# JokerYan/MS-GS

Measured on AMD Instinct MI355X. Metric: Mpixels/s fwd+bwd @1080p, 1M Gaussians; fraction of HBM roofline, higher is better.
Workload: dtype f32

## Files before the change

### ms-gs_amd/csrc/preprocess.hip

```cpp
#include "msgs_internal.h"

#include <type_traits>

#pragma clang fp contract(off)

namespace msgs {

namespace {

constexpr float SH_C0 = 0.28209479177387814f;
constexpr float SH_C1 = 0.4886025119029199f;
__device__ constexpr float SH_C2[5] = {1.0925484305920792f, -1.0925484305920792f, 0.31539156525252005f,
                                       -1.0925484305920792f, 0.5462742152960396f};
__device__ constexpr float SH_C3[7] = {-0.5900435899266435f, 2.890611442640554f, -0.4570457994644658f,
                                       0.3731763325901154f, -0.4570457994644658f, 1.445305721320277f,
                                       -0.5900435899266435f};

struct Cam {
    float V[16];
    float M[16];
    float cam[3];
};

__device__ __forceinline__ void load_cam(const ViewParams& vp, Cam& c) {
#pragma unroll
    for (int i = 0; i < 16; ++i) { c.V[i] = vp.viewmatrix[i]; c.M[i] = vp.projmatrix[i]; }
#pragma unroll
    for (int i = 0; i < 3; ++i) c.cam[i] = vp.campos[i];
}

__device__ __forceinline__ void cov3d_from_scale_rot(const float* s, float mod, const float* q, float* cov) {
    const float r = q[0], x = q[1], y = q[2], z = q[3];
    const float R[3][3] = {{1.f - 2.f * (y * y + z * z), 2.f * (x * y - r * z), 2.f * (x * z + r * y)},
                           {2.f * (x * y + r * z), 1.f - 2.f * (x * x + z * z), 2.f * (y * z - r * x)},
                           {2.f * (x * z - r * y), 2.f * (y * z + r * x), 1.f - 2.f * (x * x + y * y)}};
    const float S[3] = {mod * s[0], mod * s[1], mod * s[2]};
    float M[3][3];
#pragma unroll
    for (int i = 0; i < 3; ++i)
#pragma unroll
        for (int j = 0; j < 3; ++j) M[i][j] = R[i][j] * S[j];
    cov[0] = M[0][0] * M[0][0] + M[0][1] * M[0][1] + M[0][2] * M[0][2];
    cov[1] = M[0][0] * M[1][0] + M[0][1] * M[1][1] + M[0][2] * M[1][2];
    cov[2] = M[0][0] * M[2][0] + M[0][1] * M[2][1] + M[0][2] * M[2][2];
    cov[3] = M[1][0] * M[1][0] + M[1][1] * M[1][1] + M[1][2] * M[1][2];
    cov[4] = M[1][0] * M[2][0] + M[1][1] * M[2][1] + M[1][2] * M[2][2];
    cov[5] = M[2][0] * M[2][0] + M[2][1] * M[2][1] + M[2][2] * M[2][2];
}

struct Cov2D {
    float T[2][3];
    float a, b, c;
    float tx_c, ty_c, tz, x_mul, y_mul;
};

__device__ __forceinline__ void compute_cov2d(const float* t, const ViewParams& vp, const float* cov3D,
                                              const float* V, Cov2D& o) {
    const float limx = 1.3f * vp.tanfovx, limy = 1.3f * vp.tanfovy;
    const float txtz = t[0] / t[2], tytz = t[1] / t[2];
    o.x_mul = (txtz < -limx || txtz > limx) ? 0.f : 1.f;
    o.y_mul = (tytz < -limy || tytz > limy) ? 0.f : 1.f;
    o.tx_c = fminf(limx, fmaxf(-limx, txtz)) * t[2];
    o.ty_c = fminf(limy, fmaxf(-limy, tytz)) * t[2];
    o.tz = t[2];
    const float J[2][3] = {{vp.fx / t[2], 0.f, -(vp.fx * o.tx_c) / (t[2] * t[2])},
                           {0.f, vp.fy / t[2], -(vp.fy * o.ty_c) / (t[2] * t[2])}};
#pragma unroll
    for (int r = 0; r < 2; ++r)
#pragma unroll
        for (int c = 0; c < 3; ++c)
            o.T[r][c] = J[r][0] * V[4 * c + 0] + J[r][1] * V[4 * c + 1] + J[r][2] * V[4 * c + 2];
    const float S[3][3] = {{cov3D[0], cov3D[1], cov3D[2]}, {cov3D[1], cov3D[3], cov3D[4]},
                           {cov3D[2], cov3D[4], cov3D[5]}};
    float ST[2][3];
#pragma unroll
    for (int r = 0; r < 2; ++r)
#pragma unroll
        for (int i = 0; i < 3; ++i) ST[r][i] = S[i][0] * o.T[r][0] + S[i][1] * o.T[r][1] + S[i][2] * o.T[r][2];
    o.a = (o.T[0][0] * ST[0][0] + o.T[0][1] * ST[0][1] + o.T[0][2] * ST[0][2]) + 0.3f;
    o.b = o.T[0][0] * ST[1][0] + o.T[0][1] * ST[1][1] + o.T[0][2] * ST[1][2];
    o.c = (o.T[1][0] * ST[1][0] + o.T[1][1] * ST[1][1] + o.T[1][2] * ST[1][2]) + 0.3f;
}

__device__ __forceinline__ void view_point(const float* V, const float* p, float* t) {
    t[0] = ((V[0] * p[0] + V[4] * p[1]) + V[8] * p[2]) + V[12];
    t[1] = ((V[1] * p[0] + V[5] * p[1]) + V[9] * p[2]) + V[13];
    t[2] = ((V[2] * p[0] + V[6] * p[1]) + V[10] * p[2]) + V[14];
}

__device__ __forceinline__ void proj_point(const float* M, const float* p, float* h) {
#pragma unroll
    for (int k = 0; k < 4; ++k) h[k] = ((M[k] * p[0] + M[4 + k] * p[1]) + M[8 + k] * p[2]) + M[12 + k];
}

__device__ __forceinline__ float pixel_size_of(float opacity, float conA, float conC) {
    const float v = 255.0f * opacity;
    if (!(v > 1.0f) || !(conA > 0.f) || !(conC > 0.f)) return 0.f;
    const float ell = 2.0f * logf(v);
    const float sx = 2.0f * sqrtf(ell / conA);
    const float sy = 2.0f * sqrtf(ell / conC);
    return fminf(sx, sy);
}

__device__ __forceinline__ float filter_weight(const ViewParams& vp, float size, float minps, float maxps,
                                               bool base) {
    float w = 1.0f;
    if (vp.filter_small && !base && minps > 0.f && size < minps) {
        if (vp.fade_size > 0.f) {
            const float rel = minps / fmaxf(size, 1e-30f);
            w *= fminf(1.f, fmaxf(0.f, 1.f - (rel - 1.f) / vp.fade_size));
        } else w = 0.f;
    }
    if (vp.filter_large && maxps > 0.f && size > maxps) {
        if (vp.fade_size > 0.f) {
            const float rel = size / maxps;
            w *= fminf(1.f, fmaxf(0.f, 1.f - (rel - 1.f) / vp.fade_size));
        } else w = 0.f;
    }
    return w;
}

__device__ __forceinline__ float sh_channel(int deg, const float* sh, int c, float x, float y, float z) {
    auto S = [&](int k) { return sh[k * 3 + c]; };
    float r = SH_C0 * S(0);
    if (deg > 0) {
        r = r - SH_C1 * y * S(1) + SH_C1 * z * S(2) - SH_C1 * x * S(3);
        if (deg > 1) {
            const float xx = x * x, yy = y * y, zz = z * z, xy = x * y, yz = y * z, xz = x * z;
            r = r + SH_C2[0] * xy * S(4) + SH_C2[1] * yz * S(5) + SH_C2[2] * (2.0f * zz - xx - yy) * S(6) +
                SH_C2[3] * xz * S(7) + SH_C2[4] * (xx - yy) * S(8);
            if (deg > 2) {
                r = r + SH_C3[0] * y * (3.0f * xx - yy) * S(9) + SH_C3[1] * xy * z * S(10) +
                    SH_C3[2] * y * (4.0f * zz - xx - yy) * S(11) +
                    SH_C3[3] * z * (2.0f * zz - 3.0f * xx - 3.0f * yy) * S(12) +
                    SH_C3[4] * x * (4.0f * zz - xx - yy) * S(13) + SH_C3[5] * z * (xx - yy) * S(14) +
                    SH_C3[6] * x * (xx - 3.0f * yy) * S(15);
            }
        }
    }
    return r;
}


__device__ __forceinline__ void sh_basis(int deg, float x, float y, float z, float b[16]) {
#pragma unroll
    for (int k = 0; k < 16; ++k) b[k] = 0.f;
    b[0] = SH_C0;
    if (deg > 0) {
        b[1] = -(SH_C1 * y); b[2] = SH_C1 * z; b[3] = -(SH_C1 * x);
        if (deg > 1) {
            const float xx = x * x, yy = y * y, zz = z * z, xy = x * y, yz = y * z, xz = x * z;
            b[4] = SH_C2[0] * xy; b[5] = SH_C2[1] * yz; b[6] = SH_C2[2] * (2.0f * zz - xx - yy);
            b[7] = SH_C2[3] * xz; b[8] = SH_C2[4] * (xx - yy);
            if (deg > 2) {
                b[9] = SH_C3[0] * y * (3.0f * xx - yy); b[10] = SH_C3[1] * xy * z;
                b[11] = SH_C3[2] * y * (4.0f * zz - xx - yy);
                b[12] = SH_C3[3] * z * (2.0f * zz - 3.0f * xx - 3.0f * yy);
                b[13] = SH_C3[4] * x * (4.0f * zz - xx - yy); b[14] = SH_C3[5] * z * (xx - yy);
                b[15] = SH_C3[6] * x * (xx - 3.0f * yy);
            }
        }
    }
}

template <int K_LO, int K_HI, class F>
__device__ __forceinline__ void sh_coef_table(int deg, float x, float y, float z, F&& coef) {
    auto at = [&](int k, float basis, float bx, float by, float bz) {
        if (k >= K_LO && k < K_HI) coef(k, basis, bx, by, bz);
    };
    at(0, SH_C0, 0.f, 0.f, 0.f);
    if (deg > 0) {
        at(1, -SH_C1 * y, 0.f, -SH_C1, 0.f);
        at(2, SH_C1 * z, 0.f, 0.f, SH_C1);
        at(3, -SH_C1 * x, -SH_C1, 0.f, 0.f);
        if (deg > 1) {
            const float xx = x * x, yy = y * y, zz = z * z, xy = x * y, yz = y * z, xz = x * z;
            at(4, SH_C2[0] * xy, SH_C2[0] * y, SH_C2[0] * x, 0.f);
            at(5, SH_C2[1] * yz, 0.f, SH_C2[1] * z, SH_C2[1] * y);
            at(6, SH_C2[2] * (2.f * zz - xx - yy), SH_C2[2] * -2.f * x, SH_C2[2] * -2.f * y, SH_C2[2] * 4.f * z);
            at(7, SH_C2[3] * xz, SH_C2[3] * z, 0.f, SH_C2[3] * x);
            at(8, SH_C2[4] * (xx - yy), SH_C2[4] * 2.f * x, SH_C2[4] * -2.f * y, 0.f);
            if (deg > 2) {
                at(9, SH_C3[0] * y * (3.f * xx - yy), SH_C3[0] * 6.f * xy, SH_C3[0] * (3.f * xx - 3.f * yy), 0.f);
                at(10, SH_C3[1] * xy * z, SH_C3[1] * yz, SH_C3[1] * xz, SH_C3[1] * xy);
                at(11, SH_C3[2] * y * (4.f * zz - xx - yy), SH_C3[2] * -2.f * xy, SH_C3[2] * (4.f * zz - xx - 3.f * yy), SH_C3[2] * 8.f * yz);
                at(12, SH_C3[3] * z * (2.f * zz - 3.f * xx - 3.f * yy), SH_C3[3] * -6.f * xz, SH_C3[3] * -6.f * yz, SH_C3[3] * (6.f * zz - 3.f * xx - 3.f * yy));
                at(13, SH_C3[4] * x * (4.f * zz - xx - yy), SH_C3[4] * (4.f * zz - 3.f * xx - yy), SH_C3[4] * -2.f * xy, SH_C3[4] * 8.f * xz);
                at(14, SH_C3[5] * z * (xx - yy), SH_C3[5] * 2.f * xz, SH_C3[5] * -2.f * yz, SH_C3[5] * (xx - yy));
                at(15, SH_C3[6] * x * (xx - 3.f * yy), SH_C3[6] * (3.f * xx - 3.f * yy), SH_C3[6] * -6.f * xy, 0.f);
            }
        }
    }
}

__device__ __forceinline__ bool sh_jacobian_stored(const msgs_gaussians_t& g, const ViewParams& vp) {
    return g.raw_params != 0 || (g.shs != nullptr && vp.sh_coeffs == 16);
}

struct ShJacobian { float j[3][3]; };


template <int K_LO, int K_HI, int K_ROW>
__device__ __forceinline__ void sh_colour_accumulate(float* rgb, ShJacobian& J, int deg, float x, float y, float z,
                                                     const float* row) {
    sh_coef_table<K_LO, K_HI>(deg, x, y, z, [&](int k, float basis, float bx, float by, float bz) {
#pragma unroll
        for (int c = 0; c < 3; ++c) {
            const float v = row[3 * (k - K_ROW) + c];
            rgb[c] = rgb[c] + basis * v;
            J.j[c][0] = fmaf(bx, v, J.j[c][0]);
            J.j[c][1] = fmaf(by, v, J.j[c][1]);
            J.j[c][2] = fmaf(bz, v, J.j[c][2]);
        }
    });
}

__device__ __forceinline__ void sh_jacobian_store(char* geom, const GeomLayout& L, int P, int i, const ShJacobian& J) {
    float4* pl = reinterpret_cast<float4*>(geom + L.shjac);
    pl[i] = make_float4(J.j[0][0], J.j[0][1], J.j[0][2], J.j[1][0]);
    pl[(size_t)P + i] = make_float4(J.j[1][1], J.j[1][2], J.j[2][0], J.j[2][1]);
    reinterpret_cast<float*>(pl + 2 * (size_t)P)[i] = J.j[2][2];
}

__device__ __forceinline__ void sh_jacobian_load(const char* geom, const GeomLayout& L, int P, int i, ShJacobian& J) {
    const float4* pl = reinterpret_cast<const float4*>(geom + L.shjac);
    const float4 a = pl[i], b = pl[(size_t)P + i];
    J.j[0][0] = a.x; J.j[0][1] = a.y; J.j[0][2] = a.z; J.j[1][0] = a.w;
    J.j[1][1] = b.x; J.j[1][2] = b.y; J.j[2][0] = b.z; J.j[2][1] = b.w;
    J.j[2][2] = reinterpret_cast<const float*>(pl + 2 * (size_t)P)[i];
}

__device__ __forceinline__ void sh_ddir_from_jacobian(const ShJacobian& J, const float* g, float* ddir) {
#pragma unroll
    for (int j = 0; j < 3; ++j) ddir[j] = fmaf(J.j[2][j], g[2], fmaf(J.j[1][j], g[1], J.j[0][j] * g[0]));
}

struct ViewDir { float x, y, z, len; };
__device__ __forceinline__ ViewDir view_dir(const float* p, const float* campos) {
    const float dox = p[0] - campos[0], doy = p[1] - campos[1], doz = p[2] - campos[2];
    const float len = sqrtf(dox * dox + doy * doy + doz * doz);
    return {dox / len, doy / len, doz / len, len};
}

__device__ __forceinline__ void direction_backward(const ViewDir& d, const float* ddir, float* dm) {
    const float dotv = d.x * ddir[0] + d.y * ddir[1] + d.z * ddir[2];
    dm[0] = (ddir[0] - d.x * dotv) / d.len;
    dm[1] = (ddir[1] - d.y * dotv) / d.len;
    dm[2] = (ddir[2] - d.z * dotv) / d.len;
}

__device__ __forceinline__ void clamp_mask(float* dcolr, uint32_t fl) {
#pragma unroll
    for (int c = 0; c < 3; ++c)
        if (fl & (1u << c)) dcolr[c] = 0.f;
}

__device__ __forceinline__ void wave_lds_fence() {
    __builtin_amdgcn_fence(__ATOMIC_RELEASE, "wavefront");
    __builtin_amdgcn_wave_barrier();
    __builtin_amdgcn_fence(__ATOMIC_ACQUIRE, "wavefront");
}

constexpr int ROW_F = 48;
constexpr int ROW_LDS = 49;
constexpr int K9_STAGE_ROWS = 32;

__device__ __forceinline__ int sh_row_float4s(int deg) { return deg == 0 ? 1 : deg == 1 ? 3 : deg == 2 ? 7 : 12; }

constexpr int HALF_F4 = 6;
constexpr int HALF_LDS = 25;
__device__ __forceinline__ void coop_load_rows_part(float* lds_rows, const float* g_rows, const uint8_t* idx, int nrow,
                                                    int f4_first, int n4, int lane) {
    const int rpi = 64 / n4;
    const int sub = lane / n4, c = lane - sub * n4;
    for (int it = 0; it * rpi < nrow; ++it) {
        const int slot = it * rpi + sub;
        if (sub < rpi && slot < nrow) {
            const int sl = idx[slot];
            const float4 v = *reinterpret_cast<const float4*>(g_rows + (size_t)sl * ROW_F + 4 * (f4_first + c));
            float* d = lds_rows + sl * HALF_LDS + 4 * c;
            d[0] = v.x; d[1] = v.y; d[2] = v.z; d[3] = v.w;
        }
    }
}

__device__ __forceinline__ void coop_store_rows(const float* lds_rows, float* g_rows, int nrow, uint64_t live,
                                                int nfloat, int lane, bool acc) {
    constexpr int n4 = ROW_F / 4, rpi = 64 / n4;
    const int sub = lane / n4, c = lane - sub * n4;
    for (int it = 0; it * rpi < nrow; ++it) {
        const int row = it * rpi + sub;
        if (sub < rpi && row < nrow) {
            const bool on = (live >> row) & 1ull;
            if (acc && !on) continue;
            float4 v = make_float4(0.f, 0.f, 0.f, 0.f);
            if (on) {
                const float* sp = lds_rows + row * ROW_LDS + 4 * c;
                v.x = 4 * c + 0 < nfloat ? sp[0] : 0.f;
                v.y = 4 * c + 1 < nfloat ? sp[1] : 0.f;
                v.z = 4 * c + 2 < nfloat ? sp[2] : 0.f;
                v.w = 4 * c + 3 < nfloat ? sp[3] : 0.f;
            }
            float4* dst = reinterpret_cast<float4*>(g_rows + (size_t)row * ROW_F + 4 * c);
            if (acc) { const float4 o = *dst; v.x = o.x + v.x; v.y = o.y + v.y; v.z = o.z + v.z; v.w = o.w + v.w; }
            *dst = v;
        }
    }
}

constexpr int REST_F = 45;

__device__ __forceinline__ float act_opacity(const msgs_gaussians_t& g, int i) {
    const float x = g.opacities[i];
    return g.raw_params == 1 ? 1.0f / (1.0f + expf(-x)) : x;
}
__device__ __forceinline__ void act_scales(const msgs_gaussians_t& g, int i, float* s) {
#pragma unroll
    for (int k = 0; k < 3; ++k) { const float x = g.scales[3 * i + k]; s[k] = g.raw_params == 1 ? expf(x) : x; }
}
__device__ __forceinline__ float act_rotation(const msgs_gaussians_t& g, int i, float* q) {
    const float4 q4 = reinterpret_cast<const float4*>(g.rotations)[i];
    q[0] = q4.x; q[1] = q4.y; q[2] = q4.z; q[3] = q4.w;
    if (g.raw_params == 0) return 1.0f;
    if (g.raw_params == 2) {
        const float4 r4 = reinterpret_cast<const float4*>(g.rotations_raw)[i];
        return sqrtf(r4.x * r4.x + r4.y * r4.y + r4.z * r4.z + r4.w * r4.w);
    }
    const float rn = sqrtf(q[0] * q[0] + q[1] * q[1] + q[2] * q[2] + q[3] * q[3]);
    const float n = fmaxf(rn, 1e-12f);
#pragma unroll
    for (int k = 0; k < 4; ++k) q[k] = q[k] / n;
    return rn;
}
__device__ __forceinline__ void normalize_backward(const float* q, float rn, float* dq) {
    const float n = fmaxf(rn, 1e-12f);
    const float dotq = rn < 1e-12f ? 0.f : q[0] * dq[0] + q[1] * dq[1] + q[2] * dq[2] + q[3] * dq[3];
#pragma unroll
    for (int k = 0; k < 4; ++k) dq[k] = (dq[k] - q[k] * dotq) / n;
}

typedef float msgs_f3 __attribute__((ext_vector_type(3)));
typedef msgs_f3 __attribute__((aligned(4))) msgs_f3_u;
__device__ __forceinline__ void coop_load_split_half_listed(float* lds_rows, const float* dc, const float* rest, int wave_first,
                                                            const uint8_t* idx, int nlisted, int half, int lane) {
    const int sub = lane >> 3, c = lane & 7;
    for (int it = 0; it * 8 < nlisted; ++it) {
        const int slot = it * 8 + sub;
        if (slot < nlisted) {
            const int sl = idx[slot];
            const size_t gi = (size_t)wave_first + sl;
            float* d = lds_rows + sl * HALF_LDS + 3 * c;
            const float* src = (half == 0 && c == 0) ? dc + gi * 3 : rest + gi * 45 + 3 * (8 * half + c - 1);
            const msgs_f3 v = *reinterpret_cast<const msgs_f3_u*>(src);
            d[0] = v.x; d[1] = v.y; d[2] = v.z;
        }
    }
}

__device__ __forceinline__ void coop_load_split_rows(float* lds_rows, const float* dc, const float* rest, int i,
                                                     bool in_range, int wave_first, int nrow, int lane, int lrow) {
    if (in_range) {
#pragma unroll
        for (int c = 0; c < 3; ++c) lds_rows[lrow * ROW_LDS + c] = dc[3 * (size_t)i + c];
    }
    const float* src = rest + (size_t)wave_first * REST_F;
    const int nflat = nrow * REST_F;
    for (int base = 0; base < nflat; base += 256) {
        const int f0 = base + lane * 4;
        float v[4] = {0.f, 0.f, 0.f, 0.f};
        if (f0 + 3 < nflat) {
            const float4 t = *reinterpret_cast<const float4*>(src + f0);
            v[0] = t.x; v[1] = t.y; v[2] = t.z; v[3] = t.w;
        } else {
#pragma unroll
            for (int j = 0; j < 4; ++j) if (f0 + j < nflat) v[j] = src[f0 + j];
        }
#pragma unroll
        for (int j = 0; j < 4; ++j) {
            const int f = f0 + j;
            if (f < nflat) { const int row = f / REST_F; lds_rows[row * ROW_LDS + 3 + (f - row * REST_F)] = v[j]; }
        }
    }
}

__device__ __forceinline__ void coop_store_split_rows(const float* lds_rows, float* d_dc, float* d_rest, int i,
                                                      bool in_range, int wave_first, int nrow, uint64_t live,
                                                      int nfloat, int lane, int lrow, bool acc = false) {
    if (in_range) {
        const bool on = (live >> lrow) & 1ull;
        if (!acc) {
#pragma unroll
            for (int c = 0; c < 3; ++c) d_dc[3 * (size_t)i + c] = on ? lds_rows[lrow * ROW_LDS + c] : 0.f;
        } else if (on) {
#pragma unroll
            for (int c = 0; c < 3; ++c) d_dc[3 * (size_t)i + c] = d_dc[3 * (size_t)i + c] + lds_rows[lrow * ROW_LDS + c];
        }
    }
    float* dst = d_rest + (size_t)wave_first * REST_F;
    const int nflat = nrow * REST_F;
    for (int base = 0; base < nflat; base += 256) {
        const int f0 = base + lane * 4;
        float v[4];
        bool on[4];
#pragma unroll
        for (int j = 0; j < 4; ++j) {
            const int f = min(f0 + j, nflat - 1);
            const int row = f / REST_F, k = f - row * REST_F;
            on[j] = (live >> row) & 1ull;
            v[j] = (on[j] && 3 + k < nfloat) ? lds_rows[row * ROW_LDS + 3 + k] : 0.f;
        }
        if (f0 + 3 < nflat) {
            float4* d4 = reinterpret_cast<float4*>(dst + f0);
            if (!acc) {
                *d4 = make_float4(v[0], v[1], v[2], v[3]);
            } else if (on[0] || on[3]) {
                const float4 o = *d4;
                *d4 = make_float4(o.x + v[0], o.y + v[1], o.z + v[2], o.w + v[3]);
            }
        } else {
#pragma unroll
            for (int j = 0; j < 4; ++j)
                if (f0 + j < nflat) {
                    if (!acc) dst[f0 + j] = v[j];
                    else if (on[j]) dst[f0 + j] = dst[f0 + j] + v[j];
                }
        }
    }
}

__device__ __forceinline__ void coop_adam_split_rows(const float* lds_rows, float* p_dc, float* p_rest, const AdamInBackward& ad,
                                                     int i, bool in_range, int wave_first, int nrow, uint64_t live,
                                                     int nfloat, int lane, int lrow) {
    if (in_range) {
        const bool on = (live >> lrow) & 1ull;
#pragma unroll
        for (int c = 0; c < 3; ++c) {
            const size_t at = 3 * (size_t)i + c;
            float p = p_dc[at], m = ad.m[1][at], v = ad.v[1][at];
            adam_update(p, on ? lds_rows[lrow * ROW_LDS + c] : 0.f, m, v, ad.nss[1], ad.a);
            p_dc[at] = p; ad.m[1][at] = m; ad.v[1][at] = v;
        }
    }
    const size_t off = (size_t)wave_first * REST_F;
    float* __restrict__ P = p_rest + off;
    float* __restrict__ M = ad.m[2] + off;
    float* __restrict__ V = ad.v[2] + off;
    const float nss = ad.nss[2];
    const int nflat = nrow * REST_F;
    for (int base = 0; base < nflat; base += 256) {
        const int f0 = base + lane * 4;
        float g[4];
#pragma unroll
        for (int j = 0; j < 4; ++j) {
            const int f = min(f0 + j, nflat - 1);
            const int row = f / REST_F, k = f - row * REST_F;
            g[j] = (((live >> row) & 1ull) && 3 + k < nfloat) ? lds_rows[row * ROW_LDS + 3 + k] : 0.f;
        }
        if (f0 + 3 < nflat) {
            float4 p = *reinterpret_cast<const float4*>(P + f0), m = *reinterpret_cast<const float4*>(M + f0),
                   v = *reinterpret_cast<const float4*>(V + f0);
            adam_update(p.x, g[0], m.x, v.x, nss, ad.a);
            adam_update(p.y, g[1], m.y, v.y, nss, ad.a);
            adam_update(p.z, g[2], m.z, v.z, nss, ad.a);
            adam_update(p.w, g[3], m.w, v.w, nss, ad.a);
            *reinterpret_cast<float4*>(P + f0) = p;
            *reinterpret_cast<float4*>(M + f0) = m;
            *reinterpret_cast<float4*>(V + f0) = v;
        } else {
#pragma unroll
            for (int j = 0; j < 4; ++j)
                if (f0 + j < nflat) {
                    float p = P[f0 + j], m = M[f0 + j], v = V[f0 + j];
                    adam_update(p, g[j], m, v, nss, ad.a);
                    P[f0 + j] = p; M[f0 + j] = m; V[f0 + j] = v;
                }
        }
    }
}

template <bool SPLIT_ROWS>
__global__ __launch_bounds__(256) __attribute__((amdgpu_waves_per_eu(6))) void preprocess_kernel(ViewParams vp, msgs_gaussians_t g,
                                                         int32_t* __restrict__ radii,
                                                         float* __restrict__ pixel_sizes,
                                                         char* __restrict__ geom, ZeroJob zj,
                                                         uint32_t* __restrict__ heavy_list,
                                                         uint32_t* __restrict__ heavy_count,
                                                         uint32_t* __restrict__ heavy_blk, int write_litrec) {
    __shared__ float s_rows[4][64 * HALF_LDS];
    __shared__ uint8_t s_idx[4][64];
    __shared__ uint32_t s_heavy[4], s_hvw[4];
    const int P = g.P;
    {
        const size_t t0 = (size_t)blockIdx.x * blockDim.x + threadIdx.x, nt = (size_t)gridDim.x * blockDim.x;
        for (size_t t = t0; t < zj.n0; t += nt) zj.p0[t] = 0u;
        for (size_t t = t0; t < zj.n1; t += nt) zj.p1[t] = 0u;
    }
    const int i = blockIdx.x * blockDim.x + threadIdx.x;
    const int lane = threadIdx.x & 63, wv = threadIdx.x >> 6;
    const bool in_range = i < P;
    const GeomLayout L(P);
    GaussRec* rec = reinterpret_cast<GaussRec*>(geom + L.rec);
    BinRec* binrec = reinterpret_cast<BinRec*>(geom + L.binrec);
    uint32_t* tiles = reinterpret_cast<uint32_t*>(geom + L.tiles);
    uint32_t* key = reinterpret_cast<uint32_t*>(geom + L.key);
    uint32_t* flags = reinterpret_cast<uint32_t*>(geom + L.flags);
    float* weight = reinterpret_cast<float*>(geom + L.weight);

    Cam cm;
    load_cam(vp, cm);

    int32_t out_radius = 0;
    float out_psize = 0.f;
    uint32_t out_tiles = 0, out_cells = 0, out_key = 0xFFFFFFFFu, out_flags = 0;
    float out_weight = 0.f, out_tau2 = -3.0e38f;

    bool alive = false;
    float p[3] = {0.f, 0.f, 1.f}, t[3] = {0.f, 0.f, 0.f};
    float conA = 0.f, conB = 0.f, conC = 0.f, px = 0.f, py = 0.f, my_radius = 0.f, w = 0.f, o_eff = 0.f;
    int minx = 0, miny = 0, maxx = 0, maxy = 0;
    if (in_range) {
        p[0] = g.means3D[3 * i]; p[1] = g.means3D[3 * i + 1]; p[2] = g.means3D[3 * i + 2];
        view_point(cm.V, p, t);
    }
    do {
        if (!in_range || t[2] <= 0.2f) break;
        float h[4];
        proj_point(cm.M, p, h);
        const float pw = 1.0f / (h[3] + 0.0000001f);
        const float ndc_x = h[0] * pw, ndc_y = h[1] * pw;
        float cov3D[6];
        if (g.cov3D_precomp) {
#pragma unroll
            for (int k = 0; k < 6; ++k) cov3D[k] = g.cov3D_precomp[6 * i + k];
        } else {
            float sc[3], q[4];
            act_scales(g, i, sc);
            act_rotation(g, i, q);
            cov3d_from_scale_rot(sc, vp.scale_modifier, q, cov3D);
        }
        Cov2D c2;
        compute_cov2d(t, vp, cov3D, cm.V, c2);
        const float det = c2.a * c2.c - c2.b * c2.b;
        if (det == 0.0f) break;
        const float det_inv = 1.f / det;
        conA = c2.c * det_inv; conB = -c2.b * det_inv; conC = c2.a * det_inv;
        const float mid = 0.5f * (c2.a + c2.c);
        const float root = sqrtf(fmaxf(0.1f, mid * mid - det));
        const float lam1 = mid + root, lam2 = mid - root;
        my_radius = ceilf(3.f * sqrtf(fmaxf(lam1, lam2)));
        px = ((ndc_x + 1.0f) * vp.W - 1.0f) * 0.5f;
        py = ((ndc_y + 1.0f) * vp.H - 1.0f) * 0.5f;
        const float o = act_opacity(g, i);
        out_psize = pixel_size_of(o, conA, conC);
        minx = min(vp.gx, max(0, (int)((px - my_radius) / TILE)));
        miny = min(vp.gy, max(0, (int)((py - my_radius) / TILE)));
        maxx = min(vp.gx, max(0, (int)((px + my_radius + TILE - 1) / TILE)));
        maxy = min(vp.gy, max(0, (int)((py + my_radius + TILE - 1) / TILE)));
        if ((maxx - minx) * (maxy - miny) == 0) break;
        w = filter_weight(vp, out_psize, g.min_pixel_sizes ? g.min_pixel_sizes[i] : -1.f,
                          g.max_pixel_sizes ? g.max_pixel_sizes[i] : -1.f,
                          g.base_mask ? g.base_mask[i] != 0 : false);
        if (!(w > 0.f)) break;
        o_eff = o * w;
        alive = true;
    } while (false);

    const bool raw = g.raw_params != 0;
    const bool split_in = SPLIT_ROWS && raw && g.shs == nullptr;
    const bool staged_sh = sh_jacobian_stored(g, vp);
    float rgb[3] = {0.f, 0.f, 0.f};
    float dirx = 0.f, diry = 0.f, dirz = 0.f;
    if (alive) {
        const ViewDir d = view_dir(p, cm.cam);
        dirx = d.x; diry = d.y; dirz = d.z;
    }
    if (staged_sh) {
        const uint64_t need = __ballot(alive);
        if (alive) s_idx[wv][__popcll(need & ((1ull << lane) - 1ull))] = (uint8_t)lane;
        const int wave_first = blockIdx.x * blockDim.x + wv * 64;
        const int n4_total = sh_row_float4s(vp.sh_degree);
        ShJacobian J = {};
        for (int half = 0; half * HALF_F4 < n4_total; ++half) {
            wave_lds_fence();
            if (split_in) {
                if (need != 0)
                    coop_load_split_half_listed(s_rows[wv], g.features_dc, g.features_rest, wave_first, s_idx[wv], __popcll(need),
                                                half, lane);
            } else {
                coop_load_rows_part(s_rows[wv], g.shs + (size_t)wave_first * ROW_F, s_idx[wv], __popcll(need),
                                    half * HALF_F4, min(HALF_F4, n4_total - half * HALF_F4), lane);
            }
            wave_lds_fence();
            if (alive) {
                const float* row = (const float*)&s_rows[wv][lane * HALF_LDS];
                asm volatile("" : "+v"(dirx), "+v"(diry), "+v"(dirz));
                if (half == 0) {
                    sh_colour_accumulate<0, 4, 0>(rgb, J, vp.sh_degree, dirx, diry, dirz, row);
                    __builtin_amdgcn_sched_barrier(0);
                    sh_colour_accumulate<4, 8, 0>(rgb, J, vp.sh_degree, dirx, diry, dirz, row);
                } else {
                    sh_colour_accumulate<8, 12, 8>(rgb, J, vp.sh_degree, dirx, diry, dirz, row);
                    __builtin_amdgcn_sched_barrier(0);
                    sh_colour_accumulate<12, 16, 8>(rgb, J, vp.sh_degree, dirx, diry, dirz, row);
                }
            }
        }
        if (in_range && need != 0) sh_jacobian_store(geom, L, P, i, J);
    } else if (alive && !(g.colors_precomp && !raw)) {
        const float* sh = g.shs + (size_t)3 * vp.sh_coeffs * i;
#pragma unroll
        for (int c = 0; c < 3; ++c) rgb[c] = sh_channel(vp.sh_degree, sh, c, dirx, diry, dirz);
    }

    if (alive) {
        if (g.colors_precomp && !raw) {
#pragma unroll
            for (int c = 0; c < 3; ++c) rgb[c] = g.colors_precomp[3 * i + c];
        } else {
#pragma unroll
            for (int c = 0; c < 3; ++c) {
                float r = rgb[c] + 0.5f;
                if (r < 0.0f) { out_flags |= (1u << c); r = 0.0f; }
                rgb[c] = r;
            }
        }
        constexpr float KLOG = -0.72134752044448170368f;
        const float sA = KLOG * conA, sBh = KLOG * conB, sC = KLOG * conC;
        const float v255 = 255.0f * o_eff;
        float tau2 = 1.0f;
        uint32_t count = 0;
        const bool nd = sA < 0.f && sC < 0.f && (sA * sC - sBh * sBh) > 0.f;
        if (v255 > 1.0f) {
            tau2 = -__log2f(v255);
            tau2 = tau2 - (1e-5f * fabsf(tau2) + 2e-3f);
            if (nd) {
                const LevelSetRows ls = levelset_rows_setup(sA, sBh, sC, tau2);
                for (int ty = miny; ty < maxy; ++ty) {
                    int tlo, thi;
                    if (levelset_row_interval(ls, px, py, ty, minx, maxx, LEVELSET_MARGIN_COUNT, tlo, thi))
                        count += (uint32_t)(thi - tlo + 1);
                }
            } else {
                tau2 = -3.0e38f;
                count = (uint32_t)((maxx - minx) * (maxy - miny));
            }
        }
        if (write_litrec)
            reinterpret_cast<float4*>(geom + L.litrec)[i] = make_float4(conA, conB, conC, o_eff);
        rec[i].r0 = make_float4(px, py, sA, sBh);
        rec[i].r1 = make_float4(sC, __log2f(o_eff), rgb[0], rgb[1]);
        rec[i].r2 = make_float4(rgb[2], t[2], out_psize, tau2);
        if (count) {
            binrec[i].q0 = make_float4(px, py, sA, sBh);
            binrec[i].q1 = make_float4(sC, tau2, __uint_as_float((uint32_t)minx | ((uint32_t)miny << 16)),
                                       __uint_as_float((uint32_t)maxx | ((uint32_t)maxy << 16)));
            if (vp.cell_sx >= 0)
                out_cells = cell_range_pack(minx, miny, maxx, maxy, vp.cell_sx, vp.cell_sy) << TILE_COUNT_BITS;
        }
        out_radius = (int32_t)my_radius;
        out_tau2 = tau2;
        out_tiles = count;
        out_key = count ? __float_as_uint(t[2]) : 0xFFFFFFFFu;
        out_flags |= 8u;
        out_weight = w;
    }
    if (in_range) {
        radii[i] = out_radius;
        pixel_sizes[i] = out_psize;
        tiles[i] = out_tiles | out_cells;
        key[i] = out_key;
        flags[i] = out_flags;
        weight[i] = out_weight;
    }
    if (heavy_count) {
        const bool hv = out_tiles > OCC_HEAVY_MIN && out_tau2 > -1.0e38f;
        const uint64_t m = __ballot(hv);
        const size_t slot = (size_t)blockIdx.x * 4 + wv;
        if (hv) reinterpret_cast<uint2*>(heavy_list)[slot * 64 + __popcll(m & ((1ull << lane) - 1ull))] = make_uint2((uint32_t)i, out_key);
        uint32_t wmax = hv ? (uint32_t)(-__log2f(1.0f - fminf(0.99f, o_eff)) * 2048.0f) + 2u : 0u;
        for (int off = 32; off > 0; off >>= 1) wmax += (uint32_t)__shfl_xor((int)wmax, off);
        if (lane == 0) { heavy_count[slot] = (uint32_t)__popcll(m); s_heavy[wv] = (uint32_t)__popcll(m); s_hvw[wv] = wmax; }
        __syncthreads();
        if (threadIdx.x == 0)
            reinterpret_cast<uint2*>(heavy_blk)[blockIdx.x] = make_uint2(s_heavy[0] + s_heavy[1] + s_heavy[2] + s_heavy[3],
                                                                         min(s_hvw[0] + s_hvw[1] + s_hvw[2] + s_hvw[3], 0x0FFFFFFFu));
    }
}

__device__ __forceinline__ double (&camera_lds())[4][CAM_PARTIALS] {
    __shared__ double s[4][CAM_PARTIALS];
    return s;
}

__device__ __forceinline__ float (&camera_dir_lds())[3][256] {
    __shared__ float s[3][256];
    return s;
}

template <bool TEXTBOOK, bool ADAM, bool DEPTH = false, bool CAMERA = false>
__global__ __launch_bounds__(256) __attribute__((amdgpu_waves_per_eu(CAMERA ? 4 : 5))) void preprocess_backward_kernel(ViewParams vp, msgs_gaussians_t g,
                                                                  const int32_t* __restrict__ radii,
                                                                  const char* __restrict__ geom,
                                                                  const grad_acc_t* __restrict__ grad_rec,
                                                                  msgs_grads_t grads,
                                                                  std::conditional_t<CAMERA, CamPartials, AdamInBackward> ad) {
    static_assert(!(CAMERA && ADAM), "camera gradients are not offered with the optimizer step in the backward");
    __shared__ float s_rows[4][K9_STAGE_ROWS * ROW_LDS];
    const int P = g.P;
    const int i = blockIdx.x * blockDim.x + threadIdx.x;
    const int lane = threadIdx.x & 63, wv = threadIdx.x >> 6;
    const bool in_range = i < P;
    const GeomLayout L(P);
    const uint32_t* flags = reinterpret_cast<const uint32_t*>(geom + L.flags);
    const int K = vp.sh_coeffs;
    const int deg = vp.sh_degree;

    float dmean[3] = {0.f, 0.f, 0.f};
    float g2x = 0.f, g2y = 0.f, dopac = 0.f;
    float dcov[6] = {0.f, 0.f, 0.f, 0.f, 0.f, 0.f};
    float dcolr[3] = {0.f, 0.f, 0.f};
    float dscale[3] = {0.f, 0.f, 0.f};
    float dq[4] = {0.f, 0.f, 0.f, 0.f};
    const bool rendered = in_range && radii[i] > 0;
    const bool raw = g.raw_params != 0;
    const bool use_jac = sh_jacobian_stored(g, vp);
    const bool staged_sh = use_jac && (raw || grads.dL_dshs != nullptr);
    const bool do_colour = !g.colors_precomp;
    const bool factored_sh = !ADAM && raw && grads.dL_dfeatures_dc == nullptr;
    const bool accum = !ADAM && grads.accumulate != 0;
    const int wave_first = blockIdx.x * blockDim.x + wv * 64;
    const uint64_t live = __ballot(rendered);
    uint32_t fl = 0;
    float p[3] = {0.f, 0.f, 0.f};
    float shdm[3] = {0.f, 0.f, 0.f};
    float cdt[3] = {0.f, 0.f, 0.f}, cdh[3] = {0.f, 0.f, 0.f}, cjt[9] = {};

    if (rendered) {
        Cam cm;
        load_cam(vp, cm);
        float4 ga, gb, gc;
        if constexpr (TEXTBOOK) {
            const double* gr = reinterpret_cast<const double*>(grad_rec) + (size_t)i * (DEPTH ? DET_INST_FLOATS_DEPTH : 9);
            ga = make_float4((float)gr[0], (float)gr[1], (float)gr[2], (float)gr[3]);
            gb = make_float4((float)gr[4], (float)gr[5], (float)gr[6], (float)gr[7]);
            gc = make_float4((float)gr[8], DEPTH ? (float)gr[9] : 0.f, 0.f, 0.f);
        } else {
            const grad_acc_t* gr = grad_rec + (size_t)i * GRAD_REC_FLOATS;
            grad_acc_t t[GRAD_REC_FLOATS];
            typedef grad_acc_t acc2 __attribute__((ext_vector_type(2)));
#pragma unroll
            for (int k = 0; k < GRAD_REC_FLOATS / 2; ++k) {
                const acc2 v2 = reinterpret_cast<const acc2*>(gr)[k];
                t[2 * k] = v2.x; t[2 * k + 1] = v2.y;
            }
            ga = make_float4((float)t[0], (float)t[1], (float)t[2], (float)t[3]);
            gb = make_float4((float)t[4], (float)t[5], (float)t[6], (float)t[7]);
            gc = make_float4((float)t[8], DEPTH ? (float)t[9] : 0.f, 0.f, 0.f);
        }
        const float gA = TEXTBOOK ? ga.z : -0.5f * ga.z, gBh = TEXTBOOK ? ga.w : -0.5f * ga.w,
                    gC = TEXTBOOK ? gb.x : -0.5f * gb.x;
        const float o_in = act_opacity(g, i);
        if constexpr (TEXTBOOK)
            dopac = reinterpret_cast<const float*>(geom + L.weight)[i] * gb.y;
        else
            dopac = o_in > 0.f ? gb.y / o_in : 0.f;
        if (raw) dopac = dopac * (o_in * (1.0f - o_in));
        dcolr[0] = gb.z; dcolr[1] = gb.w; dcolr[2] = gc.x;
        fl = flags[i];
        p[0] = g.means3D[3 * i]; p[1] = g.means3D[3 * i + 1]; p[2] = g.means3D[3 * i + 2];
        if (use_jac && do_colour) {
            ShJacobian J;
            sh_jacobian_load(geom, L, P, i, J);
            clamp_mask(dcolr, fl);
            float ddir[3];
            sh_ddir_from_jacobian(J, dcolr, ddir);
            const ViewDir d = view_dir(p, vp.campos);
            direction_backward(d, ddir, shdm);
        }

        float cov3D[6];
        float R[3][3], S[3] = {0.f, 0.f, 0.f};
        float qr = 0.f, qx = 0.f, qy = 0.f, qz = 0.f, qnorm = 1.0f;
        float sact[3] = {1.f, 1.f, 1.f};
        if (g.cov3D_precomp) {
#pragma unroll
            for (int k = 0; k < 6; ++k) cov3D[k] = g.cov3D_precomp[6 * i + k];
        } else {
            float s[3], q[4];
            act_scales(g, i, s);
            qnorm = act_rotation(g, i, q);
            qr = q[0]; qx = q[1]; qy = q[2]; qz = q[3];
            sact[0] = s[0]; sact[1] = s[1]; sact[2] = s[2];
            cov3d_from_scale_rot(s, vp.scale_modifier, q, cov3D);
            S[0] = vp.scale_modifier * s[0]; S[1] = vp.scale_modifier * s[1]; S[2] = vp.scale_modifier * s[2];
            R[0][0] = 1.f - 2.f * (qy * qy + qz * qz); R[0][1] = 2.f * (qx * qy - qr * qz); R[0][2] = 2.f * (qx * qz + qr * qy);
            R[1][0] = 2.f * (qx * qy + qr * qz); R[1][1] = 1.f - 2.f * (qx * qx + qz * qz); R[1][2] = 2.f * (qy * qz - qr * qx);
            R[2][0] = 2.f * (qx * qz - qr * qy); R[2][1] = 2.f * (qy * qz + qr * qx); R[2][2] = 1.f - 2.f * (qx * qx + qy * qy);
        }

        float t[3];
        view_point(cm.V, p, t);
        Cov2D c2;
        compute_cov2d(t, vp, cov3D, cm.V, c2);
        const float ca = c2.a, cb = c2.b, cc = c2.c;
        const float denom = ca * cc - cb * cb;
        if constexpr (TEXTBOOK) {
            g2x = ga.x; g2y = ga.y;
        } else {
            constexpr float KLOG = -0.72134752044448170368f;
            constexpr float LN2 = 0.69314718055994530942f;
            const float det_inv = 1.f / denom;
            const float sA = KLOG * (cc * det_inv), sBh = KLOG * (-cb * det_inv), sC = KLOG * (ca * det_inv);
            g2x = (sA * ga.x + sBh * ga.y) * (LN2 * vp.W);
            g2y = (sC * ga.y + sBh * ga.x) * (LN2 * vp.H);
        }
        const float denom2inv = 1.0f / ((denom * denom) + 0.0000001f);
        float dL_da = 0.f, dL_db = 0.f, dL_dc = 0.f;
        if (denom2inv != 0.f) {
            dL_da = denom2inv * (-cc * cc * gA + 2 * cb * cc * gBh + (denom - ca * cc) * gC);
            dL_dc = denom2inv * (-ca * ca * gC + 2 * ca * cb * gBh + (denom - ca * cc) * gA);
            dL_db = denom2inv * 2 * (cb * cc * gA - (denom + 2 * cb * cb) * gBh + ca * cb * gC);
            const float(*T)[3] = c2.T;
            dcov[0] = T[0][0] * T[0][0] * dL_da + T[0][0] * T[1][0] * dL_db + T[1][0] * T[1][0] * dL_dc;
            dcov[3] = T[0][1] * T[0][1] * dL_da + T[0][1] * T[1][1] * dL_db + T[1][1] * T[1][1] * dL_dc;
            dcov[5] = T[0][2] * T[0][2] * dL_da + T[0][2] * T[1][2] * dL_db + T[1][2] * T[1][2] * dL_dc;
            dcov[1] = 2 * T[0][0] * T[0][1] * dL_da + (T[0][0] * T[1][1] + T[0][1] * T[1][0]) * dL_db + 2 * T[1][0] * T[1][1] * dL_dc;
            dcov[2] = 2 * T[0][0] * T[0][2] * dL_da + (T[0][0] * T[1][2] + T[0][2] * T[1][0]) * dL_db + 2 * T[1][0] * T[1][2] * dL_dc;
            dcov[4] = 2 * T[0][2] * T[0][1] * dL_da + (T[0][1] * T[1][2] + T[0][2] * T[1][1]) * dL_db + 2 * T[1][1] * T[1][2] * dL_dc;
        }
        {
            const float Sg[3][3] = {{cov3D[0], cov3D[1], cov3D[2]}, {cov3D[1], cov3D[3], cov3D[4]},
                                    {cov3D[2], cov3D[4], cov3D[5]}};
            float ST0[3], ST1[3], dT0[3], dT1[3];
#pragma unroll
            for (int k = 0; k < 3; ++k) {
                ST0[k] = Sg[k][0] * c2.T[0][0] + Sg[k][1] * c2.T[0][1] + Sg[k][2] * c2.T[0][2];
                ST1[k] = Sg[k][0] * c2.T[1][0] + Sg[k][1] * c2.T[1][1] + Sg[k][2] * c2.T[1][2];
            }
#pragma unroll
            for (int k = 0; k < 3; ++k) {
                dT0[k] = 2 * ST0[k] * dL_da + ST1[k] * dL_db;
                dT1[k] = 2 * ST1[k] * dL_dc + ST0[k] * dL_db;
            }
            const float* V = cm.V;
            const float dJ00 = V[0] * dT0[0] + V[4] * dT0[1] + V[8] * dT0[2];
            const float dJ02 = V[2] * dT0[0] + V[6] * dT0[1] + V[10] * dT0[2];
            const float dJ11 = V[1] * dT1[0] + V[5] * dT1[1] + V[9] * dT1[2];
            const float dJ12 = V[2] * dT1[0] + V[6] * dT1[1] + V[10] * dT1[2];
            const float tz = 1.f / c2.tz, tz2 = tz * tz, tz3 = tz2 * tz;
            const float dtx = c2.x_mul * -vp.fx * tz2 * dJ02;
            const float dty = c2.y_mul * -vp.fy * tz2 * dJ12;
            const float dtz = -vp.fx * tz2 * dJ00 - vp.fy * tz2 * dJ11 + (2 * vp.fx * c2.tx_c) * tz3 * dJ02 +
                              (2 * vp.fy * c2.ty_c) * tz3 * dJ12;
#pragma unroll
            for (int j = 0; j < 3; ++j) dmean[j] += V[4 * j + 0] * dtx + V[4 * j + 1] * dty + V[4 * j + 2] * dtz;
            if constexpr (CAMERA) {
                const float J00 = vp.fx / c2.tz, J02 = -(vp.fx * c2.tx_c) / (c2.tz * c2.tz);
                const float J11 = vp.fy / c2.tz, J12 = -(vp.fy * c2.ty_c) / (c2.tz * c2.tz);
                cdt[0] = dtx; cdt[1] = dty; cdt[2] = DEPTH ? dtz + gc.y : dtz;
#pragma unroll
                for (int c = 0; c < 3; ++c) {
                    cjt[3 * c + 0] = J00 * dT0[c];
                    cjt[3 * c + 1] = J11 * dT1[c];
                    cjt[3 * c + 2] = J02 * dT0[c] + J12 * dT1[c];
// ... 462 lines not shown
```

Measured before the change: 2072.

## Batch global loads ahead of use in preprocess to raise memory-level parallelism

```diff
diff --git a/ms-gs_amd/csrc/preprocess.hip b/ms-gs_amd/csrc/preprocess.hip
--- a/ms-gs_amd/csrc/preprocess.hip
+++ b/ms-gs_amd/csrc/preprocess.hip
@@ -269,19 +269,27 @@
 
 constexpr int HALF_F4 = 6;
 constexpr int HALF_LDS = 25;
+constexpr int HALF_TRIPS = (64 + 64 / HALF_F4 - 1) / (64 / HALF_F4);
 __device__ __forceinline__ void coop_load_rows_part(float* lds_rows, const float* g_rows, const uint8_t* idx, int nrow,
                                                     int f4_first, int n4, int lane) {
     const int rpi = 64 / n4;
     const int sub = lane / n4, c = lane - sub * n4;
-    for (int it = 0; it * rpi < nrow; ++it) {
+    int sl[HALF_TRIPS];
+    float4 v[HALF_TRIPS];
+#pragma unroll
+    for (int it = 0; it < HALF_TRIPS; ++it) {
         const int slot = it * rpi + sub;
-        if (sub < rpi && slot < nrow) {
-            const int sl = idx[slot];
-            const float4 v = *reinterpret_cast<const float4*>(g_rows + (size_t)sl * ROW_F + 4 * (f4_first + c));
-            float* d = lds_rows + sl * HALF_LDS + 4 * c;
-            d[0] = v.x; d[1] = v.y; d[2] = v.z; d[3] = v.w;
-        }
-    }
+        sl[it] = (sub < rpi && slot < nrow) ? (int)idx[slot] : -1;
+    }
+#pragma unroll
+    for (int it = 0; it < HALF_TRIPS; ++it)
+        if (sl[it] >= 0) v[it] = *reinterpret_cast<const float4*>(g_rows + (size_t)sl[it] * ROW_F + 4 * (f4_first + c));
+#pragma unroll
+    for (int it = 0; it < HALF_TRIPS; ++it)
+        if (sl[it] >= 0) {
+            float* d = lds_rows + sl[it] * HALF_LDS + 4 * c;
+            d[0] = v[it].x; d[1] = v[it].y; d[2] = v[it].z; d[3] = v[it].w;
+        }
 }
 
 __device__ __forceinline__ void coop_store_rows(const float* lds_rows, float* g_rows, int nrow, uint64_t live,
@@ -310,26 +318,41 @@
 
 constexpr int REST_F = 45;
 
-__device__ __forceinline__ float act_opacity(const msgs_gaussians_t& g, int i) {
-    const float x = g.opacities[i];
+__device__ __forceinline__ float opacity_activate(const msgs_gaussians_t& g, float x) {
     return g.raw_params == 1 ? 1.0f / (1.0f + expf(-x)) : x;
 }
+__device__ __forceinline__ float act_opacity(const msgs_gaussians_t& g, int i) { return opacity_activate(g, g.opacities[i]); }
+__device__ __forceinline__ void scales_load(const msgs_gaussians_t& g, int i, float* x) {
+#pragma unroll
+    for (int k = 0; k < 3; ++k) x[k] = g.scales[3 * i + k];
+}
+__device__ __forceinline__ void scales_activate(const msgs_gaussians_t& g, const float* x, float* s) {
+#pragma unroll
+    for (int k = 0; k < 3; ++k) s[k] = g.raw_params == 1 ? expf(x[k]) : x[k];
+}
 __device__ __forceinline__ void act_scales(const msgs_gaussians_t& g, int i, float* s) {
-#pragma unroll
-    for (int k = 0; k < 3; ++k) { const float x = g.scales[3 * i + k]; s[k] = g.raw_params == 1 ? expf(x) : x; }
+    float x[3];
+    scales_load(g, i, x);
+    scales_activate(g, x, s);
+}
+__device__ __forceinline__ float4 rotation_load(const msgs_gaussians_t& g, int i) {
+    return reinterpret_cast<const float4*>(g.rotations)[i];
+}
+__device__ __forceinline__ float rotation_activate(const msgs_gaussians_t& g, const float4& q4, float* q) {
+    q[0] = q4.x; q[1] = q4.y; q[2] = q4.z; q[3] = q4.w;
+    if (g.raw_params != 1) return 1.0f;
+    const float rn = sqrtf(q[0] * q[0] + q[1] * q[1] + q[2] * q[2] + q[3] * q[3]);
+    const float n = fmaxf(rn, 1e-12f);
+#pragma unroll
+    for (int k = 0; k < 4; ++k) q[k] = q[k] / n;
+    return rn;
 }
 __device__ __forceinline__ float act_rotation(const msgs_gaussians_t& g, int i, float* q) {
-    const float4 q4 = reinterpret_cast<const float4*>(g.rotations)[i];
-    q[0] = q4.x; q[1] = q4.y; q[2] = q4.z; q[3] = q4.w;
-    if (g.raw_params == 0) return 1.0f;
+    const float rn = rotation_activate(g, rotation_load(g, i), q);
     if (g.raw_params == 2) {
         const float4 r4 = reinterpret_cast<const float4*>(g.rotations_raw)[i];
         return sqrtf(r4.x * r4.x + r4.y * r4.y + r4.z * r4.z + r4.w * r4.w);
     }
-    const float rn = sqrtf(q[0] * q[0] + q[1] * q[1] + q[2] * q[2] + q[3] * q[3]);
-    const float n = fmaxf(rn, 1e-12f);
-#pragma unroll
-    for (int k = 0; k < 4; ++k) q[k] = q[k] / n;
     return rn;
 }
 __device__ __forceinline__ void normalize_backward(const float* q, float rn, float* dq) {
@@ -344,17 +367,24 @@
 __device__ __forceinline__ void coop_load_split_half_listed(float* lds_rows, const float* dc, const float* rest, int wave_first,
                                                             const uint8_t* idx, int nlisted, int half, int lane) {
     const int sub = lane >> 3, c = lane & 7;
-    for (int it = 0; it * 8 < nlisted; ++it) {
-        const int slot = it * 8 + sub;
-        if (slot < nlisted) {
-            const int sl = idx[slot];
-            const size_t gi = (size_t)wave_first + sl;
-            float* d = lds_rows + sl * HALF_LDS + 3 * c;
+    uint32_t sl[2] = {0u, 0u};
+    msgs_f3 v[8];
+#pragma unroll
+    for (int it = 0; it < 8; ++it)
+        if (it * 8 + sub < nlisted) sl[it >> 2] |= (uint32_t)idx[it * 8 + sub] << (8 * (it & 3));
+#pragma unroll
+    for (int it = 0; it < 8; ++it)
+        if (it * 8 + sub < nlisted) {
+            const size_t gi = (size_t)wave_first + ((sl[it >> 2] >> (8 * (it & 3))) & 255u);
             const float* src = (half == 0 && c == 0) ? dc + gi * 3 : rest + gi * 45 + 3 * (8 * half + c - 1);
-            const msgs_f3 v = *reinterpret_cast<const msgs_f3_u*>(src);
-            d[0] = v.x; d[1] = v.y; d[2] = v.z;
-        }
-    }
+            v[it] = *reinterpret_cast<const msgs_f3_u*>(src);
+        }
+#pragma unroll
+    for (int it = 0; it < 8; ++it)
+        if (it * 8 + sub < nlisted) {
+            float* d = lds_rows + ((sl[it >> 2] >> (8 * (it & 3))) & 255u) * HALF_LDS + 3 * c;
+            d[0] = v[it].x; d[1] = v[it].y; d[2] = v[it].z;
+        }
 }
 
 __device__ __forceinline__ void coop_load_split_rows(float* lds_rows, const float* dc, const float* rest, int i,
@@ -518,8 +548,23 @@
     float p[3] = {0.f, 0.f, 1.f}, t[3] = {0.f, 0.f, 0.f};
     float conA = 0.f, conB = 0.f, conC = 0.f, px = 0.f, py = 0.f, my_radius = 0.f, w = 0.f, o_eff = 0.f;
     int minx = 0, miny = 0, maxx = 0, maxy = 0;
+    float shape_in[7] = {0.f, 0.f, 0.f, 0.f, 0.f, 0.f, 0.f};
+    float o_in = 0.f, min_ps = -1.f, max_ps = -1.f;
+    uint8_t base_in = 0;
     if (in_range) {
         p[0] = g.means3D[3 * i]; p[1] = g.means3D[3 * i + 1]; p[2] = g.means3D[3 * i + 2];
+        if (g.cov3D_precomp) {
+#pragma unroll
+            for (int k = 0; k < 6; ++k) shape_in[k] = g.cov3D_precomp[6 * i + k];
+        } else {
+            scales_load(g, i, shape_in);
+            const float4 q4 = rotation_load(g, i);
+            shape_in[3] = q4.x; shape_in[4] = q4.y; shape_in[5] = q4.z; shape_in[6] = q4.w;
+        }
+        o_in = g.opacities[i];
+        if (g.min_pixel_sizes) min_ps = g.min_pixel_sizes[i];
+        if (g.max_pixel_sizes) max_ps = g.max_pixel_sizes[i];
+        if (g.base_mask) base_in = g.base_mask[i];
         view_point(cm.V, p, t);
     }
     do {
@@ -531,11 +576,11 @@
         float cov3D[6];
         if (g.cov3D_precomp) {
 #pragma unroll
-            for (int k = 0; k < 6; ++k) cov3D[k] = g.cov3D_precomp[6 * i + k];
+            for (int k = 0; k < 6; ++k) cov3D[k] = shape_in[k];
         } else {
             float sc[3], q[4];
-            act_scales(g, i, sc);
-            act_rotation(g, i, q);
+            scales_activate(g, shape_in, sc);
+            rotation_activate(g, make_float4(shape_in[3], shape_in[4], shape_in[5], shape_in[6]), q);
             cov3d_from_scale_rot(sc, vp.scale_modifier, q, cov3D);
         }
         Cov2D c2;
@@ -550,16 +595,14 @@
         my_radius = ceilf(3.f * sqrtf(fmaxf(lam1, lam2)));
         px = ((ndc_x + 1.0f) * vp.W - 1.0f) * 0.5f;
         py = ((ndc_y + 1.0f) * vp.H - 1.0f) * 0.5f;
-        const float o = act_opacity(g, i);
+        const float o = opacity_activate(g, o_in);
         out_psize = pixel_size_of(o, conA, conC);
         minx = min(vp.gx, max(0, (int)((px - my_radius) / TILE)));
         miny = min(vp.gy, max(0, (int)((py - my_radius) / TILE)));
         maxx = min(vp.gx, max(0, (int)((px + my_radius + TILE - 1) / TILE)));
         maxy = min(vp.gy, max(0, (int)((py + my_radius + TILE - 1) / TILE)));
         if ((maxx - minx) * (maxy - miny) == 0) break;
-        w = filter_weight(vp, out_psize, g.min_pixel_sizes ? g.min_pixel_sizes[i] : -1.f,
-                          g.max_pixel_sizes ? g.max_pixel_sizes[i] : -1.f,
-                          g.base_mask ? g.base_mask[i] != 0 : false);
+        w = filter_weight(vp, out_psize, min_ps, max_ps, base_in != 0);
         if (!(w > 0.f)) break;
         o_eff = o * w;
         alive = true;
```

Result: no change. 2078 (median of 6 runs) (+0.3%).
